# CVPR23/Depth-guided-Texture-Diffusion-for-Image-Semantic-Segmentation

Hardware: NVIDIA B200
Metric: rgbd_images_per_sec_384 (higher is better)
Workload: dtype bf16

## Files before the change

depth-guided-texture-diffusion-for-image-semantic-segmentation_b200/csrc/convnext_ops.cu:

```cuda
#include "common.cuh"

namespace dgtd {

constexpr int STEM_PX = 16;

constexpr int STEM_TILES_PER_CTA = 12;

__global__ void __launch_bounds__(256)
stem_kernel(const float* __restrict__ image, const float* __restrict__ grid, int G,
            const float* __restrict__ w, const float* __restrict__ bias,
            const float* __restrict__ ln_w, const float* __restrict__ ln_b, float* __restrict__ out,
            int H, int W, int oh, int ow, int Cout, float eps, int total_tiles) {
  extern __shared__ float sm[];
  float* in = sm;
  float* ys = sm + STEM_PX * 48;
  const int tiles_x = (ow + STEM_PX - 1) / STEM_PX;
  const int c = threadIdx.x;
  float wr[48];
#pragma unroll
  for (int k = 0; k < 48; ++k) wr[k] = w[(int64_t)c * 48 + k];
  const float bc = bias[c];
  const int lane = threadIdx.x & 31, wid = threadIdx.x >> 5, nw = blockDim.x >> 5;

  for (int it = 0; it < STEM_TILES_PER_CTA; ++it) {
// ... 283 lines not shown
  int ox = (int)(t % ow);
  t /= ow;
  int oy = (int)(t % oh), b = (int)(t / oh);
  int y0, y1, x0, x1;
  float ly, lx;
  bilinear_src(oy, (float)h / oh, h, y0, y1, ly);
  bilinear_src(ox, (float)w / ow, w, x0, x1, lx);
  const IT* xb = x + (int64_t)b * h * w * C + cq * 4;
  float4 a = load4(xb + ((int64_t)y0 * w + x0) * C), bq = load4(xb + ((int64_t)y0 * w + x1) * C);
  float4 cc = load4(xb + ((int64_t)y1 * w + x0) * C), d = load4(xb + ((int64_t)y1 * w + x1) * C);
  float w00 = (1.f - ly) * (1.f - lx), w01 = (1.f - ly) * lx, w10 = ly * (1.f - lx), w11 = ly * lx;
  store4(out + (((int64_t)b * oh + oy) * ow + ox) * C + cq * 4,
         w00 * a.x + w01 * bq.x + w10 * cc.x + w11 * d.x, w00 * a.y + w01 * bq.y + w10 * cc.y + w11 * d.y,
         w00 * a.z + w01 * bq.z + w10 * cc.z + w11 * d.z, w00 * a.w + w01 * bq.w + w10 * cc.w + w11 * d.w);
}

}

namespace dgtd {
int ln_rows_any(const float* y, const float* ln_w, const float* ln_b, void* out, int out_dtype, int64_t rows, int C,
                float eps, cudaStream_t s);
int dwconv7_ln_tma(const float* x, const float* wT, const float* dw_b, const float* ln_w, const float* ln_b,
                   float* ws, void* out, int out_dtype, int B, int h, int w, int C, float eps, cudaStream_t s);
int dwconv7_stats_tma(const float* x, const float* wT, const float* dw_b, __nv_bfloat16* y, float2* stats, int B, int h,
                      int w, int C, float eps, cudaStream_t s);
}
using namespace dgtd;

extern "C" {

int dgtd_stem_fwd(const float* image, const float* grid, int G, const float* w, const float* b,
                  const float* ln_w, const float* ln_b, float* out, int B, int H, int W, int Cout,
                  float eps, dgtd_stream_t stream) {
  DGTD_CHECK_ARG(image && w && b && ln_w && ln_b && out, "stem: null pointer");
  DGTD_CHECK_ARG(B > 0 && H >= 4 && W >= 4 && Cout >= 32 && Cout <= 256 && Cout % 32 == 0,
                 "stem: bad shape B=%d H=%d W=%d Cout=%d", B, H, W, Cout);
  DGTD_CHECK_ARG(!grid || G > 0, "stem: bad grid size");
  const int oh = H / 4, ow = W / 4;
  size_t smem = (size_t)(STEM_PX * 48 + STEM_PX * Cout) * sizeof(float);
  const int total_tiles = cdiv(ow, STEM_PX) * oh * B;
  stem_kernel<<<cdiv(total_tiles, STEM_TILES_PER_CTA), Cout, smem, (cudaStream_t)stream>>>(
      image, grid, G, w, b, ln_w, ln_b, out, H, W, oh, ow, Cout, eps, total_tiles);
  DGTD_LAUNCH_CHECK("stem");
  return 0;
}

}

// ... 72 lines not shown
               ? dwconv_launch(x, dw_w, dw_b, ln_w, ln_b, (__nv_bfloat16*)out, B, h, w, C, eps, (cudaStream_t)stream)
               : dwconv_launch(x, dw_w, dw_b, ln_w, ln_b, (float*)out, B, h, w, C, eps, (cudaStream_t)stream);
  if (rc) return rc;
  DGTD_LAUNCH_CHECK("dwconv7_ln");
  return 0;
}

int dgtd_dwconv7_ln_tma_fwd(const float* x, const float* dw_wT, const float* dw_b, const float* ln_w,
                            const float* ln_b, float* ws, void* out, int out_dtype, int B, int h, int w,
                            int C, float eps, dgtd_stream_t stream) {
  DGTD_CHECK_ARG(x && dw_wT && dw_b && ln_w && ln_b && ws && out, "dwconv7_ln_tma: null pointer");
  DGTD_CHECK_ARG(B > 0 && h > 0 && w > 0 && C >= 128 && C % 128 == 0 && C <= 1024,
                 "dwconv7_ln_tma: bad shape B=%d h=%d w=%d C=%d (C must be a multiple of 128)", B, h, w, C);
  int rc = dwconv7_ln_tma(x, dw_wT, dw_b, ln_w, ln_b, ws, out, out_dtype, B, h, w, C, eps, (cudaStream_t)stream);
  if (rc > 0) {
    set_error("dwconv7_ln_tma: shape not supported by the TMA variant");
    return -1;
  }
  if (rc) return rc;
  DGTD_LAUNCH_CHECK("dwconv7_ln_tma.ln");
  return 0;
}

int dgtd_dwconv7_stats_tma_fwd(const float* x, const float* dw_wT, const float* dw_b, void* y, float* stats, int B, int h,
                               int w, int C, float eps, dgtd_stream_t stream) {
  DGTD_CHECK_ARG(x && dw_wT && dw_b && y && stats, "dwconv7_stats_tma: null pointer");
  DGTD_CHECK_ARG(B > 0 && h > 0 && w > 0 && C >= 128 && C % 128 == 0 && C <= 1024,
                 "dwconv7_stats_tma: bad shape B=%d h=%d w=%d C=%d (C must be a multiple of 128)", B, h, w, C);
  DGTD_CHECK_ARG((reinterpret_cast<uintptr_t>(stats) & 7) == 0 && (reinterpret_cast<uintptr_t>(y) & 15) == 0,
                 "dwconv7_stats_tma: y must be 16-byte, stats 8-byte aligned");
  int rc = dwconv7_stats_tma(x, dw_wT, dw_b, (__nv_bfloat16*)y, (float2*)stats, B, h, w, C, eps, (cudaStream_t)stream);
  if (rc > 0) {
    set_error("dwconv7_stats_tma: shape not supported by the TMA variant");
    return -1;
  }
  return rc;
}

int dgtd_ln_rows_fwd(const float* y, const float* ln_w, const float* ln_b, void* out, int out_dtype, int64_t rows,
                     int C, float eps, dgtd_stream_t stream) {
  DGTD_CHECK_ARG(y && ln_w && ln_b && out && rows > 0 && C % 128 == 0 && C <= 1024, "ln_rows: bad args");
  int rc = ln_rows_any(y, ln_w, ln_b, out, out_dtype, rows, C, eps, (cudaStream_t)stream);
  if (rc) return rc;
  DGTD_LAUNCH_CHECK("ln_rows");
  return 0;
}

int dgtd_fusion_sum_fwd(const float* z0, const float* z1, const float* z2, const float* z3, const int* hw,
                        const float* bias, float* out_nhwc, float* out_nchw, void* out_pad, int Cpad, int B, int C,
                        dgtd_stream_t stream) {
  DGTD_CHECK_ARG(z0 && z1 && z2 && z3 && hw && bias, "fusion_sum: null pointer");
  DGTD_CHECK_ARG(C > 0 && C % 4 == 0, "fusion_sum: C must be a multiple of 4");
  DGTD_CHECK_ARG(out_nhwc || out_nchw || out_pad, "fusion_sum: no output requested");
  DGTD_CHECK_ARG(!out_pad || (Cpad >= C && Cpad % 4 == 0), "fusion_sum: Cpad must be a multiple of 4 and >= C");
// ... 30 lines not shown
```

depth-guided-texture-diffusion-for-image-semantic-segmentation_b200/csrc/dwconv_tma.cu:

```cuda
#include "blackwell.cuh"
#include "common.cuh"

namespace dgtd {

int sm_count();
static inline int sm_count_dw() { return sm_count(); }

template <int SY, int SX, bool ADD, typename OT = float>
__global__ void __launch_bounds__(SY * SX * 32, 2)
dwconv7_tma_kernel(const __grid_constant__ CUtensorMap tmX, const float* __restrict__ wT,
                   const float* __restrict__ bias, const float* __restrict__ add, OT* __restrict__ y, int h,
                   int w, int C, int tiles_x, int tiles_y) {
  constexpr int TH = 4 * SY, TW = 8 * SX, PH = TH + 6, PW = TW + 6, NCH = 4;
  constexpr int TILE_FLOATS = PH * PW * 32;
  constexpr uint32_t TILE_BYTES = TILE_FLOATS * 4;
  extern __shared__ __align__(128) float xs[];
  __shared__ uint64_t bar[2];

  int bid = blockIdx.x;
  const int cgs = C >> 7;
  const int cg = bid % cgs; bid /= cgs;
  const int tx = bid % tiles_x; bid /= tiles_x;
  const int ty = bid % tiles_y;
  const int b = bid / tiles_y;
// ... 86 lines not shown
      } else {
#pragma unroll
        for (int q = 0; q < 2; ++q)
#pragma unroll
          for (int j = 0; j < 8; ++j) {
            float v0, v1;
            up2(acc[q][j], v0, v1);
            if (ox0 + j < w) {
              if (oy0 + 2 * q < h) store1(yp + (2 * q) * rs + j * C, v0);
              if (oy0 + 2 * q + 1 < h) store1(yp + (2 * q + 1) * rs + j * C, v1);
            }
          }
      }
    }
    __syncthreads();
  }
}


template <int SY, int SX, bool ADD, typename OT>
__global__ void __launch_bounds__(SY * SX * 32, 2)
dwconv7_tma_persist_kernel(const __grid_constant__ CUtensorMap tmX, const __grid_constant__ CUtensorMap tmW,
                           const float* __restrict__ bias, const float* __restrict__ add, OT* __restrict__ y, int h,
                           int w, int C, int tiles_x, int tiles_y, int num_items) {
  constexpr int TH = 4 * SY, TW = 8 * SX, PH = TH + 6, PW = TW + 6;
  constexpr int TILE_FLOATS = PH * PW * 32;
  constexpr uint32_t TILE_BYTES = TILE_FLOATS * 4, W_BYTES = 49 * 32 * 4;
  extern __shared__ __align__(128) float xs[];
  float* wbuf = xs + 2 * TILE_FLOATS;
  __shared__ uint64_t bar[3];

  const int warp = threadIdx.x >> 5, lane = threadIdx.x & 31;
  const int sy = warp / SX, sx = warp - sy * SX;
  const int nch = C >> 5;
  auto issue_tile = [&](int item, int buf) {
    const int chunk = item % nch;
    int t = item / nch;
    const int tx = t % tiles_x; t /= tiles_x;
    const int ty = t % tiles_y;
    const int b = t / tiles_y;
    bw::mbar_arrive_expect_tx(&bar[buf], TILE_BYTES);
    bw::tma_load_4d(&tmX, &bar[buf], xs + buf * TILE_FLOATS, chunk * 32, tx * TW - 3, ty * TH - 3, b);
  };
  auto issue_weights = [&](int item) {
    bw::mbar_arrive_expect_tx(&bar[2], W_BYTES);
    bw::tma_load_2d(&tmW, &bar[2], wbuf, (item % nch) * 32, 0);
  };
  if (threadIdx.x == 0) {
    bw::prefetch_tmap(&tmX);
    bw::prefetch_tmap(&tmW);
    bw::mbar_init(&bar[0], 1);
    bw::mbar_init(&bar[1], 1);
    bw::mbar_init(&bar[2], 1);
    bw::fence_mbar_init();
  }
  __syncthreads();
  if (threadIdx.x == 0 && (int)blockIdx.x < num_items) {
    issue_tile(blockIdx.x, 0);
    issue_weights(blockIdx.x);
  }
  int it = 0;
#pragma unroll 1
  for (int item = blockIdx.x; item < num_items; item += gridDim.x, ++it) {
    const int next = item + gridDim.x;
    if (threadIdx.x == 0 && next < num_items) {
      bw::fence_proxy_async_smem();
      issue_tile(next, (it + 1) & 1);
    }
    const int chunk = item % nch;
    int t = item / nch;
    const int tx = t % tiles_x; t /= tiles_x;
    const int ty = t % tiles_y;
    const int b = t / tiles_y;
    const int x0 = tx * TW, y0 = ty * TH;
    const int c = chunk * 32 + lane;
    bw::mbar_wait(&bar[2], it & 1);
    uint64_t w2[49];
#pragma unroll
    for (int k = 0; k < 49; ++k) {
      const float tv = wbuf[k * 32 + lane];
      w2[k] = pk2(tv, tv);
    }
    __syncthreads();
    if (threadIdx.x == 0 && next < num_items) {
      bw::fence_proxy_async_smem();
      issue_weights(next);
    }
    const float bc = bias ? __ldg(bias + c) : 0.f;
    uint64_t acc[2][8];
#pragma unroll
    for (int q = 0; q < 2; ++q)
#pragma unroll
      for (int j = 0; j < 8; ++j) acc[q][j] = pk2(bc, bc);

    bw::mbar_wait(&bar[it & 1], (it >> 1) & 1);
    const float* base = xs + (it & 1) * TILE_FLOATS + ((4 * sy) * PW + 8 * sx) * 32 + lane;
#pragma unroll
    for (int iy = 0; iy < 9; ++iy) {
      uint64_t pr[14];
#pragma unroll
      for (int j = 0; j < 14; ++j) {
        const volatile float* p0 = base + (iy * PW + j) * 32;
        pr[j] = pk2(p0[0], p0[PW * 32]);
      }
#pragma unroll
      for (int q = 0; q < 2; ++q) {
        const int ky = iy - 2 * q;
        if (ky < 0 || ky >= 7) continue;
#pragma unroll
        for (int kx = 0; kx < 7; ++kx)
#pragma unroll
          for (int j = 0; j < 8; ++j) acc[q][j] = fma2(w2[ky * 7 + kx], pr[j + kx], acc[q][j]);
      }
    }
    if (ADD) {
      float av[4][8];
#pragma unroll
      for (int a = 0; a < 4; ++a)
#pragma unroll
        for (int j = 0; j < 8; ++j) {
          const int oy = y0 + 4 * sy + a, ox = x0 + 8 * sx + j;
          av[a][j] = (oy < h && ox < w) ? __ldg(add + (((int64_t)b * h + oy) * w + ox) * C + c) : 0.f;
        }
#pragma unroll
      for (int q = 0; q < 2; ++q)
#pragma unroll
        for (int j = 0; j < 8; ++j) acc[q][j] = add2(acc[q][j], pk2(av[2 * q][j], av[2 * q + 1][j]));
    }
    {
      const int oy0 = y0 + 4 * sy, ox0 = x0 + 8 * sx;
      OT* yp = y + (((int64_t)b * h + oy0) * w + ox0) * C + c;
      const int rs = w * C;
      if (oy0 + 4 <= h && ox0 + 8 <= w) {
#pragma unroll
        for (int q = 0; q < 2; ++q)
#pragma unroll
          for (int j = 0; j < 8; ++j) {
            float v0, v1;
            up2(acc[q][j], v0, v1);
            store1(yp + (2 * q) * rs + j * C, v0);
            store1(yp + (2 * q + 1) * rs + j * C, v1);
          }
      } else {
#pragma unroll
        for (int q = 0; q < 2; ++q)
#pragma unroll
          for (int j = 0; j < 8; ++j) {
            float v0, v1;
            up2(acc[q][j], v0, v1);
            if (ox0 + j < w) {
              if (oy0 + 2 * q < h) store1(yp + (2 * q) * rs + j * C, v0);
              if (oy0 + 2 * q + 1 < h) store1(yp + (2 * q + 1) * rs + j * C, v1);
            }
          }
      }
    }
    __syncthreads();
  }
}

template <int SY, int SX>
__global__ void __launch_bounds__(SY * SX * 32, 2)
dwconv7_wgrad_tma_kernel(const __grid_constant__ CUtensorMap tmX, const float* __restrict__ dy,
                         float* __restrict__ part, int h, int w, int C, int tiles_x, int tiles_y, int ntiles) {
  constexpr int TH = 4 * SY, TW = 8 * SX, PH = TH + 6, PW = TW + 6, NW = SY * SX;
  constexpr int TILE_FLOATS = PH * PW * 32;
  constexpr uint32_t TILE_BYTES = TILE_FLOATS * 4;
  static_assert(NW * 50 * 32 <= 2 * TILE_FLOATS, "reduction scratch must fit in the tile buffers");
  extern __shared__ __align__(128) float xs[];
  __shared__ uint64_t bar[2];

  const int chunk = blockIdx.x, P = gridDim.y;
  const int warp = threadIdx.x >> 5, lane = threadIdx.x & 31;
  const int sy = warp / SX, sx = warp - sy * SX;
  const int c = chunk * 32 + lane;

  auto issue = [&](int t, int buf) {
    const int tx = t % tiles_x;
    const int r = t / tiles_x;
    const int ty = r % tiles_y, b = r / tiles_y;
// ... 77 lines not shown
#pragma unroll
  for (int j = 0; j < VPL; ++j) {
    v[j] = *reinterpret_cast<const float4*>(p + (j * 32 + lane) * 4);
    s += (v[j].x + v[j].y) + (v[j].z + v[j].w);
  }
  const float mean = warp_sum(s) / C;
  float q = 0.f;
#pragma unroll
  for (int j = 0; j < VPL; ++j) {
    float a = v[j].x - mean, b = v[j].y - mean, c = v[j].z - mean, d = v[j].w - mean;
    q += (a * a + b * b) + (c * c + d * d);
  }
  const float rstd = 1.0f / sqrtf(warp_sum(q) / C + eps);
  OT* o = out + row * C;
#pragma unroll
  for (int j = 0; j < VPL; ++j) {
    const int c0 = (j * 32 + lane) * 4;
    float4 g = *reinterpret_cast<const float4*>(ln_w + c0), be = *reinterpret_cast<const float4*>(ln_b + c0);
    store4(o + c0, (v[j].x - mean) * rstd * g.x + be.x, (v[j].y - mean) * rstd * g.y + be.y,
           (v[j].z - mean) * rstd * g.z + be.z, (v[j].w - mean) * rstd * g.w + be.w);
  }
}

template <int LPR, int V, int U>
__global__ void __launch_bounds__(256)
row_stats_bf16_kernel(const __nv_bfloat16* __restrict__ y, float2* __restrict__ stats, int64_t rows, int C, float eps) {
  constexpr int RPP = 32 / LPR;
  constexpr int RPW = RPP * U;
  const int lane = threadIdx.x & 31, sub = lane / LPR, l = lane % LPR;
  const int64_t row0 = ((int64_t)blockIdx.x * 8 + (threadIdx.x >> 5)) * RPW + sub;
  uint4 raw[U][V];
#pragma unroll
  for (int u = 0; u < U; ++u) {
    const int64_t row = row0 + u * RPP;
#pragma unroll
    for (int j = 0; j < V; ++j) {
      raw[u][j] = make_uint4(0u, 0u, 0u, 0u);
      if (row < rows) raw[u][j] = __ldg(reinterpret_cast<const uint4*>(y + row * C + (j * LPR + l) * 8));
    }
  }
  const float inv_c = 1.0f / C;
#pragma unroll
  for (int u = 0; u < U; ++u) {
    float f[V][8];
    float s = 0.f;
#pragma unroll
    for (int j = 0; j < V; ++j) {
      const uint32_t w4[4] = {raw[u][j].x, raw[u][j].y, raw[u][j].z, raw[u][j].w};
#pragma unroll
      for (int e = 0; e < 4; ++e) {
        f[j][2 * e] = __uint_as_float(w4[e] << 16);
        f[j][2 * e + 1] = __uint_as_float(w4[e] & 0xffff0000u);
      }
      s += ((f[j][0] + f[j][1]) + (f[j][2] + f[j][3])) + ((f[j][4] + f[j][5]) + (f[j][6] + f[j][7]));
    }
#pragma unroll
    for (int o = LPR / 2; o > 0; o >>= 1) s += __shfl_xor_sync(0xffffffffu, s, o);
    const float mean = s * inv_c;
    float q = 0.f;
#pragma unroll
    for (int j = 0; j < V; ++j) {
#pragma unroll
      for (int e = 0; e < 8; e += 2) {
        const float a = f[j][e] - mean, b = f[j][e + 1] - mean;
        q += a * a + b * b;
      }
    }
#pragma unroll
    for (int o = LPR / 2; o > 0; o >>= 1) q += __shfl_xor_sync(0xffffffffu, q, o);
    const int64_t row = row0 + u * RPP;
    if (l == 0 && row < rows) stats[row] = make_float2(mean, 1.0f / sqrtf(q * inv_c + eps));
  }
}

static int row_stats_grid(int64_t rows, int rows_per_block) { return (int)cdiv(rows, rows_per_block); }

int row_stats_bf16(const __nv_bfloat16* y, float2* stats, int64_t rows, int C, float eps, cudaStream_t s) {
  if (reinterpret_cast<uintptr_t>(y) & 15) {
    set_error("row_stats: the matrix must be 16-byte aligned");
    return -1;
  }
  switch (C / 128) {
    case 1: row_stats_bf16_kernel<16, 1, 4><<<row_stats_grid(rows, 64), 256, 0, s>>>(y, stats, rows, C, eps); break;
    case 2: row_stats_bf16_kernel<32, 1, 4><<<row_stats_grid(rows, 32), 256, 0, s>>>(y, stats, rows, C, eps); break;
    case 4: row_stats_bf16_kernel<32, 2, 2><<<row_stats_grid(rows, 16), 256, 0, s>>>(y, stats, rows, C, eps); break;
    case 8: row_stats_bf16_kernel<32, 4, 1><<<row_stats_grid(rows, 8), 256, 0, s>>>(y, stats, rows, C, eps); break;
    default:
      set_error("row_stats: C=%d must be 128*{1,2,4,8}", C);
      return -1;
  }
  return 0;
}

template <int SY, int SX, bool ADD, typename OT>
static int dw_launch_persist(const CUtensorMap& tm, const float* wT, const float* bias, const float* add, OT* y, int B, int h,
                             int w, int C, cudaStream_t s) {
  constexpr int PH = 4 * SY + 6, PW = 8 * SX + 6;
  constexpr int SMEM = 2 * PH * PW * 128 + 49 * 32 * 4 + 128;
  auto kern = dwconv7_tma_persist_kernel<SY, SX, ADD, OT>;
  static bool configured = false;
  if (!configured) {
    cudaError_t e = cudaFuncSetAttribute(kern, cudaFuncAttributeMaxDynamicSharedMemorySize, SMEM);
    if (e != cudaSuccess) {
      set_error("dwconv7_tma(persistent): cannot opt in to %d B smem: %s", SMEM, cudaGetErrorString(e));
      return -2;
    }
    configured = true;
  }
  CUtensorMap tmW;
  {
    const uint64_t dims[2] = {(uint64_t)C, 49}, strides[1] = {(uint64_t)C * 4};
    const uint32_t box[2] = {32, 49};
    int rc = make_tmap(&tmW, wT, CU_TENSOR_MAP_DATA_TYPE_FLOAT32, 2, dims, strides, box, CU_TENSOR_MAP_SWIZZLE_NONE);
    if (rc) return rc;
  }
  const int tiles_x = cdiv(w, 8 * SX), tiles_y = cdiv(h, 4 * SY);
  const int64_t items = (int64_t)B * tiles_x * tiles_y * (C / 32);
  if (items > 0x7fffffff) {
    set_error("dwconv7_tma(persistent): too many items");
    return -1;
  }
  const int slots = 2 * sm_count_dw();
  const int grid = items < slots ? (int)items : slots;
  kern<<<grid, SY * SX * 32, SMEM, s>>>(tm, tmW, bias, add, y, h, w, C, tiles_x, tiles_y, (int)items);
  return 0;
}

template <int SY, int SX>
static int dw_launch_bf16(const CUtensorMap& tm, const float* wT, const float* bias, __nv_bfloat16* y, int B, int h, int w,
                          int C, cudaStream_t s) {
  if ((reinterpret_cast<uintptr_t>(wT) & 15) == 0)
    return dw_launch_persist<SY, SX, false, __nv_bfloat16>(tm, wT, bias, nullptr, y, B, h, w, C, s);
  constexpr int PH = 4 * SY + 6, PW = 8 * SX + 6;
  constexpr int SMEM = 2 * PH * PW * 128 + 128;
  auto kern = dwconv7_tma_kernel<SY, SX, false, __nv_bfloat16>;
  static bool configured = false;
  if (!configured) {
    cudaError_t e = cudaFuncSetAttribute(kern, cudaFuncAttributeMaxDynamicSharedMemorySize, SMEM);
    if (e != cudaSuccess) {
      set_error("dwconv7_tma(bf16): cannot opt in to %d B smem: %s", SMEM, cudaGetErrorString(e));
      return -2;
    }
    configured = true;
  }
  const int tiles_x = cdiv(w, 8 * SX), tiles_y = cdiv(h, 4 * SY);
  const int64_t blocks = (int64_t)B * tiles_x * tiles_y * (C / 128);
  kern<<<(unsigned)blocks, SY * SX * 32, SMEM, s>>>(tm, wT, bias, nullptr, y, h, w, C, tiles_x, tiles_y);
  return 0;
}

template <int SY, int SX>
static int dw_launch(const CUtensorMap& tm, const float* wT, const float* bias, const float* add, float* y, int B,
                     int h, int w, int C, cudaStream_t s) {
  if ((reinterpret_cast<uintptr_t>(wT) & 15) == 0) {
    if (add) return dw_launch_persist<SY, SX, true, float>(tm, wT, bias, add, y, B, h, w, C, s);
    return dw_launch_persist<SY, SX, false, float>(tm, wT, bias, nullptr, y, B, h, w, C, s);
  }
  constexpr int PH = 4 * SY + 6, PW = 8 * SX + 6;
  constexpr int SMEM = 2 * PH * PW * 128 + 128;
  static bool configured = false;
  if (!configured) {
    cudaError_t e = cudaFuncSetAttribute(dwconv7_tma_kernel<SY, SX, false>, cudaFuncAttributeMaxDynamicSharedMemorySize, SMEM);
    if (e == cudaSuccess)
      e = cudaFuncSetAttribute(dwconv7_tma_kernel<SY, SX, true>, cudaFuncAttributeMaxDynamicSharedMemorySize, SMEM);
    if (e != cudaSuccess) {
      set_error("dwconv7_tma: cannot opt in to %d B smem: %s", SMEM, cudaGetErrorString(e));
      return -2;
    }
    configured = true;
  }
// ... 110 lines not shown
  const int ntiles = B * cdiv(w, 8 * SX) * cdiv(h, 4 * SY);
  int P = cdiv(2 * 148, C / 32);
  if (P > ntiles) P = ntiles;
  if (P > max_parts) P = max_parts;
  if (P < 1) return 1;
  CUtensorMap tm;
  int rc = dw_make_tmap(&tm, x, B, h, w, C, SY, SX);
  if (rc) return rc;
  if (SY == 2 && SX == 2) rc = dwg_launch<2, 2>(tm, dy, part, P, B, h, w, C, s);
  else if (SY == 2 && SX == 3) rc = dwg_launch<2, 3>(tm, dy, part, P, B, h, w, C, s);
  else if (SY == 3 && SX == 2) rc = dwg_launch<3, 2>(tm, dy, part, P, B, h, w, C, s);
  else rc = dwg_launch<3, 3>(tm, dy, part, P, B, h, w, C, s);
  if (rc) return rc;
  cudaError_t e = cudaGetLastError();
  if (e != cudaSuccess) {
    set_error("dwconv7_wgrad_tma: launch failed: %s", cudaGetErrorString(e));
    return -2;
  }
  count_launch();
  *parts = P;
  return 0;
}

int dwconv7_stats_tma(const float* x, const float* wT, const float* dw_b, __nv_bfloat16* y, float2* stats, int B, int h,
                      int w, int C, float eps, cudaStream_t s) {
  if (C % 128 || C > 1024 || (reinterpret_cast<uintptr_t>(x) & 15)) return 1;
  int SY, SX;
  dw_tile_shape(h, w, &SY, &SX);
  CUtensorMap tm;
  int rc = dw_make_tmap(&tm, x, B, h, w, C, SY, SX);
  if (rc) return rc;
  if (SY == 2 && SX == 2) rc = dw_launch_bf16<2, 2>(tm, wT, dw_b, y, B, h, w, C, s);
  else if (SY == 2 && SX == 3) rc = dw_launch_bf16<2, 3>(tm, wT, dw_b, y, B, h, w, C, s);
  else if (SY == 3 && SX == 2) rc = dw_launch_bf16<3, 2>(tm, wT, dw_b, y, B, h, w, C, s);
  else rc = dw_launch_bf16<3, 3>(tm, wT, dw_b, y, B, h, w, C, s);
  if (rc) return rc;
  cudaError_t e = cudaGetLastError();
  if (e != cudaSuccess) {
    set_error("dwconv7_stats_tma: launch failed: %s", cudaGetErrorString(e));
    return -2;
  }
  count_launch();
  rc = row_stats_bf16(y, stats, (int64_t)B * h * w, C, eps, s);
  if (rc) return rc;
  e = cudaGetLastError();
  if (e != cudaSuccess) {
    set_error("row_stats: launch failed: %s", cudaGetErrorString(e));
    return -2;
  }
  count_launch();
  return 0;
}

int dwconv7_ln_tma(const float* x, const float* wT, const float* dw_b, const float* ln_w, const float* ln_b,
                   float* ws, void* out, int out_dtype, int B, int h, int w, int C, float eps, cudaStream_t s) {
  int rc = dwconv7_tma(x, wT, dw_b, nullptr, ws, B, h, w, C, s);
  if (rc) return rc;
  const int64_t rows = (int64_t)B * h * w;
  return out_dtype == DGTD_BF16 ? ln_rows_launch(ws, ln_w, ln_b, (__nv_bfloat16*)out, rows, C, eps, s)
                                : ln_rows_launch(ws, ln_w, ln_b, (float*)out, rows, C, eps, s);
}

int ln_rows_any(const float* y, const float* ln_w, const float* ln_b, void* out, int out_dtype, int64_t rows, int C,
                float eps, cudaStream_t s) {
  return out_dtype == DGTD_BF16 ? ln_rows_launch(y, ln_w, ln_b, (__nv_bfloat16*)out, rows, C, eps, s)
                                : ln_rows_launch(y, ln_w, ln_b, (float*)out, rows, C, eps, s);
}

}
```

depth-guided-texture-diffusion-for-image-semantic-segmentation_b200/twig/ops/capi.py:

```python
from __future__ import annotations

import ctypes
import os
from ctypes import c_char_p, c_float, c_int, c_int64, c_void_p
from typing import Optional

import torch

_HERE = os.path.dirname(os.path.abspath(__file__))
LIB_PATH = os.path.join(_HERE, "libdgtd_ops.so")

F32, BF16 = 0, 1
ACT_NONE, ACT_GELU, ACT_RELU = 0, 1, 2

_P, _I, _L, _F = c_void_p, c_int, c_int64, c_float

SIGNATURES = {
    "dgtd_version": [],
    "dgtd_last_error": [],
    "dgtd_launch_count": [],
    "dgtd_surface_normals_fwd": [_P, _P, _I, _I, _I, _P],
    "dgtd_lowpass_projector": [_P, _P, _I, _I, _P],
    "dgtd_fft_highpass_fwd": [_P, _P, _P, _P, _P, _P, _P, _P, _I, _I, _I, _P],
    "dgtd_fft_highpass_tc3_fwd": [_P, _P, _P, _P, _P, _P, _P, _P, _P, _I, _I, _I, _P],
    "dgtd_diffusion_front_fwd": [_P] * 11 + [_I] * 6 + [_P],
    "dgtd_message_passing_fwd": [_P, _P, _P, _P, _I, _I, _I, _I, _I, _I, _F, _P],
    "dgtd_message_passing_tiled_fwd": [_P, _P, _P, _P, _I, _I, _I, _I, _I, _F, _I, _P],
    "dgtd_message_passing_tiled_simt_fwd": [_P, _P, _P, _P, _I, _I, _I, _I, _I, _F, _I, _P],
    "dgtd_message_passing_tc_fwd": [_P, _P, _P, _P, _I, _I, _I, _I, _I, _F, _I, _P],
    "dgtd_pack_regressor": [_P, _P, _P, _I, _P],
    "dgtd_message_passing_regress_fwd": [_P, _P, _P, _P, _P, _I, _I, _I, _I, _I, _F, _I, _I, _P],
    "dgtd_message_passing_bwd": [_P, _P, _P, _P, _P, _I, _I, _I, _I, _I, _I, _F, _P],
    "dgtd_conv1x1_nchw_fwd": [_P, _P, _P, _P, _I, _I, _I, _I, _I, _P],
    "dgtd_conv1x1_nchw_bwd": [_P, _P, _P, _P, _P, _P, _P, _I, _I, _I, _I, _P],
    "dgtd_resize_bilinear_nchw_bwd": [_P, _P, _I, _I, _I, _I, _I, _P],
    "dgtd_resize_nchw_fwd": [_P, _P, _I, _I, _I, _I, _I, _I, _P],
    "dgtd_resize_sigmoid_sized_fwd": [_P, _P, _P, _I, _I, _I, _I, _I, _P],
    "dgtd_layer_norm_fwd": [_P, _P, _P, _P, _L, _I, _L, _F, _P],
    "dgtd_stem_fwd": [_P, _P, _I, _P, _P, _P, _P, _P, _I, _I, _I, _I, _F, _P],
    "dgtd_ln_patchify_fwd": [_P, _P, _P, _P, _I, _I, _I, _I, _I, _F, _P],
    "dgtd_dwconv7_ln_fwd": [_P, _P, _P, _P, _P, _P, _I, _I, _I, _I, _I, _F, _P],
    "dgtd_dwconv7_ln_tma_fwd": [_P, _P, _P, _P, _P, _P, _P, _I, _I, _I, _I, _I, _F, _P],
    "dgtd_linear_fwd": [_P, _P, _P, _P, _I, _I, _I, _I, _I, _I, _I, _P],
    "dgtd_dwconv7_stats_tma_fwd": [_P, _P, _P, _P, _P, _I, _I, _I, _I, _F, _P],
    "dgtd_linear_ln_fwd": [_P, _P, _P, _P, _P, _F, _P, _I, _I, _I, _P],
    "dgtd_linear_tf32_fwd": [_P, _P, _P, _P, _I, _I, _I, _I, _P],
    "dgtd_linear_lnfold_fwd": [_P, _P, _P, _P, _P, _P, _I, _I, _I, _I, _I, _I, _P],
    "dgtd_linear_residual_fwd": [_P, _P, _P, _P, _P, _I, _P, _P, _I, _I, _I, _I, _P],
    "dgtd_convnext_mlp_fused_fwd": [_P, _P, _P, _P, _P, _P, _P, _P, _P, _P, _L, _I, _P],
    "dgtd_fusion_sum_fwd": [_P, _P, _P, _P, _P, _P, _P, _P, _P, _I, _I, _I, _P],
    "dgtd_conv_nhwc_fwd": [_P, _P, _P, _P] + [_I] * 15 + [_P],
    "dgtd_conv_nhwc_grouped_fwd": [_P, _P, _P, _P] + [_I] * 16 + [_L, _I, _L, _P],
    "dgtd_resize_nhwc_fwd": [_P, _P, _I, _I, _I, _I, _I, _I, _I, _I, _P],
    "dgtd_linear_dgrad": [_P, _P, _P, _P, _P, _P, _I, _I, _I, _I, _I, _P],
    "dgtd_linear_wgrad": [_P, _P, _P, _P, _P] + [_I] * 13 + [_P],
    "dgtd_linear_wgrad_ws_floats": [_I, _I, _I],
    "dgtd_colsum": [_P, _P, _I, _P, _P, _I, _I, _P],
    "dgtd_layer_scale_finalize": [_P, _P, _P, _P, _P, _P, _P, _P, _I, _I, _P],
    "dgtd_gelu_fwd": [_P, _P, _L, _P],
    "dgtd_relu_bwd": [_P, _P, _P, _L, _P],
    "dgtd_ln_rows_bwd": [_P, _P, _P, _P, _P, _P, _P, _L, _I, _F, _P],
    "dgtd_ln_rows_bwd_ws_floats": [_L, _I],
    "dgtd_dwconv7_fwd": [_P, _P, _P, _P, _P, _I, _I, _I, _I, _I, _P],
    "dgtd_dwconv7_wgrad": [_P, _P, _P, _P, _P, _I, _I, _I, _I, _P],
    "dgtd_stem_patchify": [_P, _P, _I, _P, _I, _I, _I, _I, _P],
    "dgtd_stem_unpatchify": [_P, _P, _I, _I, _I, _P],
    "dgtd_patchify2": [_P, _P, _I, _I, _I, _I, _P],
# ... 159 lines not shown
```

depth-guided-texture-diffusion-for-image-semantic-segmentation_b200/twig/ops/functions/texture_diffusion_func.py:

```python
from __future__ import annotations

from typing import List, Optional, Sequence, Tuple

import torch
from torch.autograd import Function
from torch.autograd.function import once_differentiable

from .. import capi
from ..capi import ACT_GELU, ACT_NONE, ACT_RELU, BF16, F32, call, check_cuda, ptr, stream

__all__ = [
    "surface_normals", "HighpassPlan", "fft_highpass", "diffusion_front", "MessagePassingFunction",
    "message_passing_core", "message_passing_tiled", "conv1x1_nchw_autograd", "resize_bilinear_nchw_autograd", "conv1x1_nchw", "resize_nchw", "layer_norm",
    "stem", "stem_patches", "ln_rows_", "fusion_sum", "ln_patchify", "dwconv7_ln", "dwconv7_ln_tma", "linear", "linear_ln", "linear_tf32", "linear_residual_", "conv_nhwc", "conv_nhwc_grouped",
    "resize_nhwc", "cast", "nhwc_to_nchw", "nchw_to_nhwc", "enable_gemm_profile", "collect_gemm_profile",
]


_PROFILE = {"on": False, "events": []}


def enable_gemm_profile(on: bool = True):
    _PROFILE["on"] = bool(on)
    _PROFILE["events"] = []
    return _PROFILE
# ... 284 lines not shown
    return out


def dwconv7_ln(x: torch.Tensor, dw_w, dw_b, ln_w, ln_b, out_dtype: int, eps: float = 1e-6) -> torch.Tensor:
    check_cuda(x, dw_w, dw_b, ln_w, ln_b)
    B, h, w, C = x.shape
    out = torch.empty(B, h, w, C, device=x.device, dtype=_tdtype(out_dtype))
    call("dgtd_dwconv7_ln_fwd", ptr(x), ptr(dw_w), ptr(dw_b), ptr(ln_w), ptr(ln_b), ptr(out), out_dtype, B, h,
         w, C, float(eps), stream())
    return out


def dwconv7_ln_tma(x: torch.Tensor, dw_wT, dw_b, ln_w, ln_b, out_dtype: int, ws: torch.Tensor,
                   eps: float = 1e-6) -> torch.Tensor:
    check_cuda(x, dw_wT, dw_b, ln_w, ln_b, ws)
    B, h, w, C = x.shape
    assert ws.numel() >= x.numel() and ws.dtype == torch.float32
    out = torch.empty(B, h, w, C, device=x.device, dtype=_tdtype(out_dtype))
    call("dgtd_dwconv7_ln_tma_fwd", ptr(x), ptr(dw_wT), ptr(dw_b), ptr(ln_w), ptr(ln_b), ptr(ws), ptr(out),
         out_dtype, B, h, w, C, float(eps), stream())
    return out


def dwconv7_stats_tma(x: torch.Tensor, dw_wT, dw_b, eps: float = 1e-6):
    check_cuda(x, dw_wT, dw_b)
    B, h, w, C = x.shape
    y = torch.empty(B, h, w, C, device=x.device, dtype=torch.bfloat16)
    stats = torch.empty(B * h * w, 2, device=x.device, dtype=torch.float32)
    call("dgtd_dwconv7_stats_tma_fwd", ptr(x), ptr(dw_wT), ptr(dw_b), ptr(y), ptr(stats), B, h, w, C, float(eps), stream())
    return y, stats


def linear_lnfold(a: torch.Tensor, w: torch.Tensor, bias: torch.Tensor, col_s: torch.Tensor, row_stats: torch.Tensor,
                  act: int = ACT_NONE, out_dtype: int = BF16) -> torch.Tensor:
    check_cuda(a, w, bias, col_s, row_stats)
    K = a.shape[-1]
    M = a.numel() // K
    N = w.shape[0]
    assert w.shape[1] == K and a.dtype == torch.bfloat16 and w.dtype == torch.bfloat16 and row_stats.shape == (M, 2)
    out = torch.empty(tuple(a.shape[:-1]) + (N,), device=a.device, dtype=_tdtype(out_dtype))
    with _timed(2.0 * M * N * K, True, (M, N, K)):
        call("dgtd_linear_lnfold_fwd", ptr(a), ptr(w), ptr(bias), ptr(col_s), ptr(row_stats), ptr(out), M, N, K, N,
             out_dtype, act, stream())
    return out


def linear(a: torch.Tensor, w: torch.Tensor, bias: Optional[torch.Tensor], act: int = ACT_NONE,
           out_dtype: Optional[int] = None, out: Optional[torch.Tensor] = None) -> torch.Tensor:
    check_cuda(a, w, bias)
    K = a.shape[-1]
    M = a.numel() // K
    N = w.shape[0]
# ... 163 lines not shown
```

include/dgtd_ops.h:

```cpp
#ifndef DGTD_OPS_H_
#define DGTD_OPS_H_

#include <stddef.h>
#include <stdint.h>

#ifdef __cplusplus
extern "C" {
#endif

#define DGTD_VERSION 100
#define DGTD_F32 0
#define DGTD_BF16 1

#define DGTD_ACT_NONE 0
#define DGTD_ACT_GELU 1
#define DGTD_ACT_RELU 2

typedef void* dgtd_stream_t;

int dgtd_version(void);
const char* dgtd_last_error(void);
int64_t dgtd_launch_count(void);

int dgtd_surface_normals_fwd(const float* depth, float* normals, int B, int H, int W,
// ... 40 lines not shown
                          dgtd_stream_t stream);
int dgtd_resize_bilinear_nchw_bwd(const float* grad_out, float* grad_x, int planes, int h, int w, int oh,
                                  int ow, dgtd_stream_t stream);
int dgtd_resize_nchw_fwd(const float* x, float* out, int planes, int h, int w, int oh, int ow,
                         int bilinear, dgtd_stream_t stream);
int dgtd_resize_sigmoid_sized_fwd(const float* x, float* out, const int32_t* sizes, int B, int h, int w, int Hmax,
                                  int Wmax, dgtd_stream_t stream);
int dgtd_layer_norm_fwd(const float* x, const float* w, const float* b, float* out, int64_t outer,
                        int C, int64_t inner, float eps, dgtd_stream_t stream);

int dgtd_stem_fwd(const float* image, const float* grid, int G, const float* w, const float* b,
                  const float* ln_w, const float* ln_b, float* out, int B, int H, int W, int Cout,
                  float eps, dgtd_stream_t stream);
int dgtd_ln_patchify_fwd(const float* x, const float* ln_w, const float* ln_b, void* out,
                         int out_dtype, int B, int h, int w, int C, float eps,
                         dgtd_stream_t stream);

int dgtd_dwconv7_ln_fwd(const float* x, const float* dw_w, const float* dw_b, const float* ln_w,
                        const float* ln_b, void* out, int out_dtype, int B, int h, int w, int C,
                        float eps, dgtd_stream_t stream);
int dgtd_dwconv7_ln_tma_fwd(const float* x, const float* dw_wT, const float* dw_b, const float* ln_w,
                            const float* ln_b, float* ws, void* out, int out_dtype, int B, int h, int w,
                            int C, float eps, dgtd_stream_t stream);
int dgtd_dwconv7_stats_tma_fwd(const float* x, const float* dw_wT, const float* dw_b, void* y, float* stats, int B,
                               int h, int w, int C, float eps, dgtd_stream_t stream);
int dgtd_linear_ln_fwd(const void* a, const void* w, const float* bias, const float* ln_w, const float* ln_b, float eps,
                       float* out, int M, int N, int K, dgtd_stream_t stream);
int dgtd_linear_tf32_fwd(const float* a, const float* w, const float* bias, float* out, int M, int N, int K, int ldo,
                         dgtd_stream_t stream);
int dgtd_linear_lnfold_fwd(const void* a, const void* w, const float* bias, const float* col_s, const float* row_stats,
                           void* out, int M, int N, int K, int ldo, int dtype_out, int act, dgtd_stream_t stream);
int dgtd_convnext_mlp_fused_fwd(const void* y, const float* row_stats, const void* w1, const float* col_s,
                                const float* cbias, const void* w2, const float* b2, const float* gamma,
                                const float* residual, float* out, int64_t M, int C, dgtd_stream_t stream);
int dgtd_linear_fwd(const void* a, const void* w, const float* bias, void* out, int M, int N,
                    int K, int ldo, int dtype_in, int dtype_out, int act, dgtd_stream_t stream);
int dgtd_linear_residual_fwd(const void* a, const void* w, const float* bias, const float* gamma,
                             const float* keep, int rows_per_sample, const float* residual,
                             float* out, int M, int N, int K, int dtype_in, dgtd_stream_t stream);

int dgtd_fusion_sum_fwd(const float* z0, const float* z1, const float* z2, const float* z3, const int* hw,
                        const float* bias, float* out_nhwc, float* out_nchw, void* out_pad, int Cpad, int B, int C,
                        dgtd_stream_t stream);

int dgtd_conv_nhwc_fwd(const void* x, const void* w, const float* bias, void* out, int B, int h,
                       int wd, int Cin, int ldx, int oh, int ow, int Cout, int ldo, int ks,
                       int stride, int off, int act, int dtype_in, int dtype_out,
                       dgtd_stream_t stream);
// ... 161 lines not shown
```

Before: 5346.

## Fuse per-pixel LayerNorm statistics into persistent bf16 depthwise-conv kernel

The bf16 depthwise 7x7 conv now computes per-chunk partial sums and centered second moments for each pixel, writes them to a scratch buffer, and uses per-subtile atomic counters so the last-arriving chunk merges them into mean/rstd. This removes the separate row_stats kernel launch and its re-read of the bf16 output. The output is staged through swizzled shared memory for vectorized stores. The next-tile TMA prefetch is moved after the barrier so the staging buffer can be reused. The change adds atomics, fences, a deferred merge step, and a persistent counter buffer that must return to zero. The non-persistent fallback for misaligned weights is dropped.

Result: slower. 4572, median of 6 (-14.5%).

```diff
diff --git a/depth-guided-texture-diffusion-for-image-semantic-segmentation_b200/csrc/convnext_ops.cu b/depth-guided-texture-diffusion-for-image-semantic-segmentation_b200/csrc/convnext_ops.cu
--- a/depth-guided-texture-diffusion-for-image-semantic-segmentation_b200/csrc/convnext_ops.cu
+++ b/depth-guided-texture-diffusion-for-image-semantic-segmentation_b200/csrc/convnext_ops.cu
@@ -329,8 +329,8 @@
                 float eps, cudaStream_t s);
 int dwconv7_ln_tma(const float* x, const float* wT, const float* dw_b, const float* ln_w, const float* ln_b,
                    float* ws, void* out, int out_dtype, int B, int h, int w, int C, float eps, cudaStream_t s);
-int dwconv7_stats_tma(const float* x, const float* wT, const float* dw_b, __nv_bfloat16* y, float2* stats, int B, int h,
-                      int w, int C, float eps, cudaStream_t s);
+int dwconv7_stats_tma(const float* x, const float* wT, const float* dw_b, __nv_bfloat16* y, float2* stats, float2* part,
+                      unsigned* counters, int B, int h, int w, int C, float eps, cudaStream_t s);
 }
 using namespace dgtd;
 
@@ -449,14 +449,16 @@
   return 0;
 }
 
-int dgtd_dwconv7_stats_tma_fwd(const float* x, const float* dw_wT, const float* dw_b, void* y, float* stats, int B, int h,
-                               int w, int C, float eps, dgtd_stream_t stream) {
-  DGTD_CHECK_ARG(x && dw_wT && dw_b && y && stats, "dwconv7_stats_tma: null pointer");
+int dgtd_dwconv7_stats_tma_fwd(const float* x, const float* dw_wT, const float* dw_b, void* y, float* stats, float* part,
+                               unsigned* counters, int B, int h, int w, int C, float eps, dgtd_stream_t stream) {
+  DGTD_CHECK_ARG(x && dw_wT && dw_b && y && stats && part && counters, "dwconv7_stats_tma: null pointer");
   DGTD_CHECK_ARG(B > 0 && h > 0 && w > 0 && C >= 128 && C % 128 == 0 && C <= 1024,
                  "dwconv7_stats_tma: bad shape B=%d h=%d w=%d C=%d (C must be a multiple of 128)", B, h, w, C);
-  DGTD_CHECK_ARG((reinterpret_cast<uintptr_t>(stats) & 7) == 0 && (reinterpret_cast<uintptr_t>(y) & 15) == 0,
-                 "dwconv7_stats_tma: y must be 16-byte, stats 8-byte aligned");
-  int rc = dwconv7_stats_tma(x, dw_wT, dw_b, (__nv_bfloat16*)y, (float2*)stats, B, h, w, C, eps, (cudaStream_t)stream);
+  DGTD_CHECK_ARG((reinterpret_cast<uintptr_t>(stats) & 7) == 0 && (reinterpret_cast<uintptr_t>(part) & 7) == 0 &&
+                     (reinterpret_cast<uintptr_t>(y) & 15) == 0 && (reinterpret_cast<uintptr_t>(dw_wT) & 15) == 0,
+                 "dwconv7_stats_tma: y and dw_wT must be 16-byte, stats and part 8-byte aligned");
+  int rc = dwconv7_stats_tma(x, dw_wT, dw_b, (__nv_bfloat16*)y, (float2*)stats, (float2*)part, counters, B, h, w, C, eps,
+                             (cudaStream_t)stream);
   if (rc > 0) {
     set_error("dwconv7_stats_tma: shape not supported by the TMA variant");
     return -1;
diff --git a/depth-guided-texture-diffusion-for-image-semantic-segmentation_b200/csrc/dwconv_tma.cu b/depth-guided-texture-diffusion-for-image-semantic-segmentation_b200/csrc/dwconv_tma.cu
--- a/depth-guided-texture-diffusion-for-image-semantic-segmentation_b200/csrc/dwconv_tma.cu
+++ b/depth-guided-texture-diffusion-for-image-semantic-segmentation_b200/csrc/dwconv_tma.cu
@@ -1,3 +1,5 @@
+#include <type_traits>
+
 #include "blackwell.cuh"
 #include "common.cuh"
 
@@ -132,7 +134,9 @@
 __global__ void __launch_bounds__(SY * SX * 32, 2)
 dwconv7_tma_persist_kernel(const __grid_constant__ CUtensorMap tmX, const __grid_constant__ CUtensorMap tmW,
                            const float* __restrict__ bias, const float* __restrict__ add, OT* __restrict__ y, int h,
-                           int w, int C, int tiles_x, int tiles_y, int num_items) {
+                           int w, int C, int tiles_x, int tiles_y, int num_items, float2* __restrict__ part,
+                           unsigned* __restrict__ counters, float2* __restrict__ stats, float eps) {
+  constexpr bool STATS = std::is_same<OT, __nv_bfloat16>::value;
   constexpr int TH = 4 * SY, TW = 8 * SX, PH = TH + 6, PW = TW + 6;
   constexpr int TILE_FLOATS = PH * PW * 32;
   constexpr uint32_t TILE_BYTES = TILE_FLOATS * 4, W_BYTES = 49 * 32 * 4;
@@ -143,6 +147,57 @@
   const int warp = threadIdx.x >> 5, lane = threadIdx.x & 31;
   const int sy = warp / SX, sx = warp - sy * SX;
   const int nch = C >> 5;
+  const int sub_x = (w + 7) >> 3, sub_y = (h + 3) >> 2;
+  auto sub_tile = [&](int item, int& b, int& oy0, int& ox0) {
+    int t = item / nch;
+    const int tx = t % tiles_x; t /= tiles_x;
+    const int ty = t % tiles_y;
+    b = t / tiles_y;
+    oy0 = ty * TH + 4 * sy;
+    ox0 = tx * TW + 8 * sx;
+    return (oy0 < h && ox0 < w) ? (b * sub_y + (oy0 >> 2)) * sub_x + (ox0 >> 3) : -1;
+  };
+  auto arrive = [&](int item) -> unsigned {
+    int b, oy0, ox0;
+    const int sub = sub_tile(item, b, oy0, ox0);
+    unsigned old = 0;
+    if (lane == 0 && sub >= 0)
+      asm volatile("atom.release.gpu.global.add.u32 %0, [%1], 1;" : "=r"(old) : "l"(counters + sub) : "memory");
+    return old;
+  };
+  auto merge = [&](int item, unsigned old) {
+    int b, oy0, ox0;
+    const int sub = sub_tile(item, b, oy0, ox0);
+    if (sub < 0 || __shfl_sync(0xffffffffu, old, 0) != (unsigned)(nch - 1)) return;
+    if (lane == 0) counters[sub] = 0u;
+    asm volatile("fence.acq_rel.gpu;" ::: "memory");
+    __syncwarp();
+    const int oy = oy0 + (lane >> 3), ox = ox0 + (lane & 7);
+    if (oy >= h || ox >= w) return;
+    const int64_t pix = ((int64_t)b * h + oy) * w + ox;
+    const float2* pp = part + pix * nch;
+    float2 pv[32];
+#pragma unroll
+    for (int k = 0; k < 32; ++k)
+      if (k < nch) pv[k] = __ldcg(pp + k);
+    const float inv_c = 1.0f / C;
+    float s = 0.f;
+#pragma unroll
+    for (int k = 0; k < 32; ++k)
+      if (k < nch) s += pv[k].x;
+    const float mean = s * inv_c;
+    float m2 = 0.f, dev = 0.f;
+#pragma unroll
+    for (int k = 0; k < 32; ++k)
+      if (k < nch) {
+        const float d = pv[k].x * (1.0f / 32) - mean;
+        m2 += pv[k].y;
+        dev += d * d;
+      }
+    m2 += 32.f * dev;
+    stats[pix] = make_float2(mean, 1.0f / sqrtf(m2 * inv_c + eps));
+  };
+  int pend = -1;
   auto issue_tile = [&](int item, int buf) {
     const int chunk = item % nch;
     int t = item / nch;
@@ -173,7 +228,7 @@
 #pragma unroll 1
   for (int item = blockIdx.x; item < num_items; item += gridDim.x, ++it) {
     const int next = item + gridDim.x;
-    if (threadIdx.x == 0 && next < num_items) {
+    if (!STATS && threadIdx.x == 0 && next < num_items) {
       bw::fence_proxy_async_smem();
       issue_tile(next, (it + 1) & 1);
     }
@@ -194,6 +249,7 @@
     __syncthreads();
     if (threadIdx.x == 0 && next < num_items) {
       bw::fence_proxy_async_smem();
+      if (STATS) issue_tile(next, (it + 1) & 1);
       issue_weights(next);
     }
     const float bc = bias ? __ldg(bias + c) : 0.f;
@@ -237,7 +293,61 @@
 #pragma unroll
         for (int j = 0; j < 8; ++j) acc[q][j] = add2(acc[q][j], pk2(av[2 * q][j], av[2 * q + 1][j]));
     }
-    {
+    if constexpr (STATS) {
+      const unsigned pend_old = pend >= 0 ? arrive(pend) : 0u;
+      __syncthreads();
+      uint32_t* stg = reinterpret_cast<uint32_t*>(xs + (it & 1) * TILE_FLOATS) + warp * 512;
+#pragma unroll
+      for (int q = 0; q < 2; ++q)
+#pragma unroll
+        for (int j = 0; j < 8; ++j) {
+          float v0, v1;
+          up2(acc[q][j], v0, v1);
+          const __nv_bfloat162 r = __floats2bfloat162_rn(v0, v1);
+          stg[(8 * q + j) * 32 + ((((lane >> 2) ^ j) << 2) | (lane & 3))] = *reinterpret_cast<const uint32_t*>(&r);
+        }
+      __syncwarp();
+      const int pp = lane & 15, hf = lane >> 4;
+      const unsigned sel = hf ? 0x7632u : 0x5410u;
+      uint32_t yw[16];
+#pragma unroll
+      for (int g = 0; g < 8; ++g) {
+        const uint4 r = *reinterpret_cast<const uint4*>(stg + pp * 32 + ((g ^ (pp & 7)) << 2));
+        yw[2 * g] = __byte_perm(r.x, r.y, sel);
+        yw[2 * g + 1] = __byte_perm(r.z, r.w, sel);
+      }
+      bw::fence_proxy_async_smem();
+      const int oy = y0 + 4 * sy + 2 * (pp >> 3) + hf, ox = x0 + 8 * sx + (pp & 7);
+      if (oy < h && ox < w) {
+        const int64_t pix = ((int64_t)b * h + oy) * w + ox;
+        uint4* yp = reinterpret_cast<uint4*>(y + pix * C + chunk * 32);
+#pragma unroll
+        for (int k = 0; k < 4; ++k) yp[k] = make_uint4(yw[4 * k], yw[4 * k + 1], yw[4 * k + 2], yw[4 * k + 3]);
+        uint64_t f[16];
+#pragma unroll
+        for (int m = 0; m < 16; ++m) f[m] = pk2(__uint_as_float(yw[m] << 16), __uint_as_float(yw[m] & 0xffff0000u));
+        uint64_t s2[2] = {f[0], f[1]};
+#pragma unroll
+        for (int m = 2; m < 16; ++m) s2[m & 1] = add2(s2[m & 1], f[m]);
+        float sa, sb, sc, sd;
+        up2(s2[0], sa, sb);
+        up2(s2[1], sc, sd);
+        const float sum = (sa + sb) + (sc + sd);
+        const float nm = -sum * (1.0f / 32);
+        const uint64_t nm2 = pk2(nm, nm);
+        uint64_t q2[2] = {0ull, 0ull};
+#pragma unroll
+        for (int m = 0; m < 16; ++m) {
+          const uint64_t d = add2(f[m], nm2);
+          q2[m & 1] = fma2(d, d, q2[m & 1]);
+        }
+        up2(q2[0], sa, sb);
+        up2(q2[1], sc, sd);
+        part[pix * nch + chunk] = make_float2(sum, (sa + sb) + (sc + sd));
+      }
+      if (pend >= 0) merge(pend, pend_old);
+      pend = item;
+    } else {
       const int oy0 = y0 + 4 * sy, ox0 = x0 + 8 * sx;
       OT* yp = y + (((int64_t)b * h + oy0) * w + ox0) * C + c;
       const int rs = w * C;
@@ -264,8 +374,12 @@
             }
           }
       }
-    }
-    __syncthreads();
+      __syncthreads();
+    }
+  }
+  if (STATS && pend >= 0) {
+    __syncwarp();
+    merge(pend, arrive(pend));
   }
 }
 
@@ -389,79 +503,10 @@
   }
 }
 
-template <int LPR, int V, int U>
-__global__ void __launch_bounds__(256)
-row_stats_bf16_kernel(const __nv_bfloat16* __restrict__ y, float2* __restrict__ stats, int64_t rows, int C, float eps) {
-  constexpr int RPP = 32 / LPR;
-  constexpr int RPW = RPP * U;
-  const int lane = threadIdx.x & 31, sub = lane / LPR, l = lane % LPR;
-  const int64_t row0 = ((int64_t)blockIdx.x * 8 + (threadIdx.x >> 5)) * RPW + sub;
-  uint4 raw[U][V];
-#pragma unroll
-  for (int u = 0; u < U; ++u) {
-    const int64_t row = row0 + u * RPP;
-#pragma unroll
-    for (int j = 0; j < V; ++j) {
-      raw[u][j] = make_uint4(0u, 0u, 0u, 0u);
-      if (row < rows) raw[u][j] = __ldg(reinterpret_cast<const uint4*>(y + row * C + (j * LPR + l) * 8));
-    }
-  }
-  const float inv_c = 1.0f / C;
-#pragma unroll
-  for (int u = 0; u < U; ++u) {
-    float f[V][8];
-    float s = 0.f;
-#pragma unroll
-    for (int j = 0; j < V; ++j) {
-      const uint32_t w4[4] = {raw[u][j].x, raw[u][j].y, raw[u][j].z, raw[u][j].w};
-#pragma unroll
-      for (int e = 0; e < 4; ++e) {
-        f[j][2 * e] = __uint_as_float(w4[e] << 16);
-        f[j][2 * e + 1] = __uint_as_float(w4[e] & 0xffff0000u);
-      }
-      s += ((f[j][0] + f[j][1]) + (f[j][2] + f[j][3])) + ((f[j][4] + f[j][5]) + (f[j][6] + f[j][7]));
-    }
-#pragma unroll
-    for (int o = LPR / 2; o > 0; o >>= 1) s += __shfl_xor_sync(0xffffffffu, s, o);
-    const float mean = s * inv_c;
-    float q = 0.f;
-#pragma unroll
-    for (int j = 0; j < V; ++j) {
-#pragma unroll
-      for (int e = 0; e < 8; e += 2) {
-        const float a = f[j][e] - mean, b = f[j][e + 1] - mean;
-        q += a * a + b * b;
-      }
-    }
-#pragma unroll
-    for (int o = LPR / 2; o > 0; o >>= 1) q += __shfl_xor_sync(0xffffffffu, q, o);
-    const int64_t row = row0 + u * RPP;
-    if (l == 0 && row < rows) stats[row] = make_float2(mean, 1.0f / sqrtf(q * inv_c + eps));
-  }
-}
-
-static int row_stats_grid(int64_t rows, int rows_per_block) { return (int)cdiv(rows, rows_per_block); }
-
-int row_stats_bf16(const __nv_bfloat16* y, float2* stats, int64_t rows, int C, float eps, cudaStream_t s) {
-  if (reinterpret_cast<uintptr_t>(y) & 15) {
-    set_error("row_stats: the matrix must be 16-byte aligned");
-    return -1;
-  }
-  switch (C / 128) {
-    case 1: row_stats_bf16_kernel<16, 1, 4><<<row_stats_grid(rows, 64), 256, 0, s>>>(y, stats, rows, C, eps); break;
-    case 2: row_stats_bf16_kernel<32, 1, 4><<<row_stats_grid(rows, 32), 256, 0, s>>>(y, stats, rows, C, eps); break;
-    case 4: row_stats_bf16_kernel<32, 2, 2><<<row_stats_grid(rows, 16), 256, 0, s>>>(y, stats, rows, C, eps); break;
-    case 8: row_stats_bf16_kernel<32, 4, 1><<<row_stats_grid(rows, 8), 256, 0, s>>>(y, stats, rows, C, eps); break;
-    default:
-      set_error("row_stats: C=%d must be 128*{1,2,4,8}", C);
-      return -1;
-  }
-  return 0;
-}
-
 template <int SY, int SX, bool ADD, typename OT>
 static int dw_launch_persist(const CUtensorMap& tm, const float* wT, const float* bias, const float* add, OT* y, int B, int h,
-                             int w, int C, cudaStream_t s) {
+                             int w, int C, cudaStream_t s, float2* part = nullptr, unsigned* counters = nullptr,
+                             float2* stats = nullptr, float eps = 0.f) {
   constexpr int PH = 4 * SY + 6, PW = 8 * SX + 6;
   constexpr int SMEM = 2 * PH * PW * 128 + 49 * 32 * 4 + 128;
   auto kern = dwconv7_tma_persist_kernel<SY, SX, ADD, OT>;
@@ -489,30 +534,8 @@
   }
   const int slots = 2 * sm_count_dw();
   const int grid = items < slots ? (int)items : slots;
-  kern<<<grid, SY * SX * 32, SMEM, s>>>(tm, tmW, bias, add, y, h, w, C, tiles_x, tiles_y, (int)items);
-  return 0;
-}
-
-template <int SY, int SX>
-static int dw_launch_bf16(const CUtensorMap& tm, const float* wT, const float* bias, __nv_bfloat16* y, int B, int h, int w,
-                          int C, cudaStream_t s) {
-  if ((reinterpret_cast<uintptr_t>(wT) & 15) == 0)
-    return dw_launch_persist<SY, SX, false, __nv_bfloat16>(tm, wT, bias, nullptr, y, B, h, w, C, s);
-  constexpr int PH = 4 * SY + 6, PW = 8 * SX + 6;
-  constexpr int SMEM = 2 * PH * PW * 128 + 128;
-  auto kern = dwconv7_tma_kernel<SY, SX, false, __nv_bfloat16>;
-  static bool configured = false;
-  if (!configured) {
-    cudaError_t e = cudaFuncSetAttribute(kern, cudaFuncAttributeMaxDynamicSharedMemorySize, SMEM);
-    if (e != cudaSuccess) {
-      set_error("dwconv7_tma(bf16): cannot opt in to %d B smem: %s", SMEM, cudaGetErrorString(e));
-      return -2;
-    }
-    configured = true;
-  }
-  const int tiles_x = cdiv(w, 8 * SX), tiles_y = cdiv(h, 4 * SY);
-  const int64_t blocks = (int64_t)B * tiles_x * tiles_y * (C / 128);
-  kern<<<(unsigned)blocks, SY * SX * 32, SMEM, s>>>(tm, wT, bias, nullptr, y, h, w, C, tiles_x, tiles_y);
+  kern<<<grid, SY * SX * 32, SMEM, s>>>(tm, tmW, bias, add, y, h, w, C, tiles_x, tiles_y, (int)items, part, counters,
+                                         stats, eps);
   return 0;
 }
 
@@ -669,30 +692,23 @@
   return 0;
 }
 
-int dwconv7_stats_tma(const float* x, const float* wT, const float* dw_b, __nv_bfloat16* y, float2* stats, int B, int h,
-                      int w, int C, float eps, cudaStream_t s) {
+int dwconv7_stats_tma(const float* x, const float* wT, const float* dw_b, __nv_bfloat16* y, float2* stats, float2* part,
+                      unsigned* counters, int B, int h, int w, int C, float eps, cudaStream_t s) {
   if (C % 128 || C > 1024 || (reinterpret_cast<uintptr_t>(x) & 15)) return 1;
   int SY, SX;
   dw_tile_shape(h, w, &SY, &SX);
   CUtensorMap tm;
   int rc = dw_make_tmap(&tm, x, B, h, w, C, SY, SX);
   if (rc) return rc;
-  if (SY == 2 && SX == 2) rc = dw_launch_bf16<2, 2>(tm, wT, dw_b, y, B, h, w, C, s);
-  else if (SY == 2 && SX == 3) rc = dw_launch_bf16<2, 3>(tm, wT, dw_b, y, B, h, w, C, s);
-  else if (SY == 3 && SX == 2) rc = dw_launch_bf16<3, 2>(tm, wT, dw_b, y, B, h, w, C, s);
-  else rc = dw_launch_bf16<3, 3>(tm, wT, dw_b, y, B, h, w, C, s);
+  using bf = __nv_bfloat16;
+  if (SY == 2 && SX == 2) rc = dw_launch_persist<2, 2, false, bf>(tm, wT, dw_b, nullptr, y, B, h, w, C, s, part, counters, stats, eps);
+  else if (SY == 2 && SX == 3) rc = dw_launch_persist<2, 3, false, bf>(tm, wT, dw_b, nullptr, y, B, h, w, C, s, part, counters, stats, eps);
+  else if (SY == 3 && SX == 2) rc = dw_launch_persist<3, 2, false, bf>(tm, wT, dw_b, nullptr, y, B, h, w, C, s, part, counters, stats, eps);
+  else rc = dw_launch_persist<3, 3, false, bf>(tm, wT, dw_b, nullptr, y, B, h, w, C, s, part, counters, stats, eps);
   if (rc) return rc;
   cudaError_t e = cudaGetLastError();
   if (e != cudaSuccess) {
     set_error("dwconv7_stats_tma: launch failed: %s", cudaGetErrorString(e));
-    return -2;
-  }
-  count_launch();
-  rc = row_stats_bf16(y, stats, (int64_t)B * h * w, C, eps, s);
-  if (rc) return rc;
-  e = cudaGetLastError();
-  if (e != cudaSuccess) {
-    set_error("row_stats: launch failed: %s", cudaGetErrorString(e));
     return -2;
   }
   count_launch();
diff --git a/depth-guided-texture-diffusion-for-image-semantic-segmentation_b200/twig/ops/capi.py b/depth-guided-texture-diffusion-for-image-semantic-segmentation_b200/twig/ops/capi.py
--- a/depth-guided-texture-diffusion-for-image-semantic-segmentation_b200/twig/ops/capi.py
+++ b/depth-guided-texture-diffusion-for-image-semantic-segmentation_b200/twig/ops/capi.py
@@ -42,7 +42,7 @@
     "dgtd_dwconv7_ln_fwd": [_P, _P, _P, _P, _P, _P, _I, _I, _I, _I, _I, _F, _P],
     "dgtd_dwconv7_ln_tma_fwd": [_P, _P, _P, _P, _P, _P, _P, _I, _I, _I, _I, _I, _F, _P],
     "dgtd_linear_fwd": [_P, _P, _P, _P, _I, _I, _I, _I, _I, _I, _I, _P],
-    "dgtd_dwconv7_stats_tma_fwd": [_P, _P, _P, _P, _P, _I, _I, _I, _I, _F, _P],
+    "dgtd_dwconv7_stats_tma_fwd": [_P, _P, _P, _P, _P, _P, _P, _I, _I, _I, _I, _F, _P],
     "dgtd_linear_ln_fwd": [_P, _P, _P, _P, _P, _F, _P, _I, _I, _I, _P],
     "dgtd_linear_tf32_fwd": [_P, _P, _P, _P, _I, _I, _I, _I, _P],
     "dgtd_linear_lnfold_fwd": [_P, _P, _P, _P, _P, _P, _I, _I, _I, _I, _I, _I, _P],
diff --git a/depth-guided-texture-diffusion-for-image-semantic-segmentation_b200/twig/ops/functions/texture_diffusion_func.py b/depth-guided-texture-diffusion-for-image-semantic-segmentation_b200/twig/ops/functions/texture_diffusion_func.py
--- a/depth-guided-texture-diffusion-for-image-semantic-segmentation_b200/twig/ops/functions/texture_diffusion_func.py
+++ b/depth-guided-texture-diffusion-for-image-semantic-segmentation_b200/twig/ops/functions/texture_diffusion_func.py
@@ -1,6 +1,6 @@
 from __future__ import annotations
 
-from typing import List, Optional, Sequence, Tuple
+from typing import Dict, List, Optional, Sequence, Tuple
 
 import torch
 from torch.autograd import Function
@@ -331,12 +331,29 @@
     return out
 
 
+_STATS_COUNTERS: Dict[tuple, torch.Tensor] = {}
+
+
+def _stats_counters(device: torch.device, numel: int) -> torch.Tensor:
+    if torch.cuda.is_current_stream_capturing():
+        return torch.zeros(numel, device=device, dtype=torch.int32)
+    key = (device, torch.cuda.current_stream(device).cuda_stream)
+    buf = _STATS_COUNTERS.get(key)
+    if buf is None or buf.numel() < numel:
+        buf = _STATS_COUNTERS[key] = torch.zeros(numel, device=device, dtype=torch.int32)
+    return buf
+
+
 def dwconv7_stats_tma(x: torch.Tensor, dw_wT, dw_b, eps: float = 1e-6):
+    from ...model.texture_diffuser import scratch_buffer
     check_cuda(x, dw_wT, dw_b)
     B, h, w, C = x.shape
     y = torch.empty(B, h, w, C, device=x.device, dtype=torch.bfloat16)
     stats = torch.empty(B * h * w, 2, device=x.device, dtype=torch.float32)
-    call("dgtd_dwconv7_stats_tma_fwd", ptr(x), ptr(dw_wT), ptr(dw_b), ptr(y), ptr(stats), B, h, w, C, float(eps), stream())
+    part = scratch_buffer("dw_stats_part", x.device, B * h * w * (C // 32) * 2, torch.float32)
+    counters = _stats_counters(x.device, B * ((h + 3) // 4) * ((w + 7) // 8))
+    call("dgtd_dwconv7_stats_tma_fwd", ptr(x), ptr(dw_wT), ptr(dw_b), ptr(y), ptr(stats), ptr(part), ptr(counters),
+         B, h, w, C, float(eps), stream())
     return y, stats
 
 
diff --git a/include/dgtd_ops.h b/include/dgtd_ops.h
--- a/include/dgtd_ops.h
+++ b/include/dgtd_ops.h
@@ -86,8 +86,8 @@
 int dgtd_dwconv7_ln_tma_fwd(const float* x, const float* dw_wT, const float* dw_b, const float* ln_w,
                             const float* ln_b, float* ws, void* out, int out_dtype, int B, int h, int w,
                             int C, float eps, dgtd_stream_t stream);
-int dgtd_dwconv7_stats_tma_fwd(const float* x, const float* dw_wT, const float* dw_b, void* y, float* stats, int B,
-                               int h, int w, int C, float eps, dgtd_stream_t stream);
+int dgtd_dwconv7_stats_tma_fwd(const float* x, const float* dw_wT, const float* dw_b, void* y, float* stats, float* part,
+                               unsigned* counters, int B, int h, int w, int C, float eps, dgtd_stream_t stream);
 int dgtd_linear_ln_fwd(const void* a, const void* w, const float* bias, const float* ln_w, const float* ln_b, float eps,
                        float* out, int M, int N, int K, dgtd_stream_t stream);
 int dgtd_linear_tf32_fwd(const float* a, const float* w, const float* bias, float* out, int M, int N, int K, int ldo,
```
